# urbste/MultiCol-SLAM

Measured on AMD Instinct MI355X. Metric: Mfeatures/s extract+match, 3-cam 754x480 multi-frame, higher is better.
Workload: dtype u8+i32 (images, Hamming) / f64 (omni model)

## Files before the change

multicol-slam_amd/csrc/mcs_fast.hip:

```cpp
#include "mcs_common.h"

#include <algorithm>
#include <cstdio>
#include <cstdlib>

namespace mcs {

#ifndef MCS_FAST_BS
#define MCS_FAST_BS 128
#endif
template <int CW> struct FastGeom {
	static constexpr int kTileX = 4;
	static constexpr int kTilePitch = (CW + kTileX + 3 + 4 + 3) / 4 * 4, kTileRows = CW + 6;
	static constexpr int kScPitch = (CW + 2 + 3) / 4 * 4, kScRows = CW + 2;
};

template <int P, int kTilePitch> struct Ring;
template <int kTilePitch> struct Ring<12, kTilePitch> {
	static __device__ __forceinline__ void diffs(const uint8_t* c, int (&d)[12]) {
		const int v = c[0];
		d[0] = v - c[2 * kTilePitch]; d[1] = v - c[2 * kTilePitch + 1]; d[2] = v - c[kTilePitch + 2]; d[3] = v - c[2];
		d[4] = v - c[-kTilePitch + 2]; d[5] = v - c[-2 * kTilePitch + 1]; d[6] = v - c[-2 * kTilePitch]; d[7] = v - c[-2 * kTilePitch - 1];
		d[8] = v - c[-kTilePitch - 2]; d[9] = v - c[-2]; d[10] = v - c[kTilePitch - 2]; d[11] = v - c[2 * kTilePitch - 1];
	}
};
template <int kTilePitch> struct Ring<8, kTilePitch> {
	static __device__ __forceinline__ void diffs(const uint8_t* c, int (&d)[8]) {
		const int v = c[0];
		d[0] = v - c[kTilePitch]; d[1] = v - c[kTilePitch + 1]; d[2] = v - c[1]; d[3] = v - c[-kTilePitch + 1];
		d[4] = v - c[-kTilePitch]; d[5] = v - c[-kTilePitch - 1]; d[6] = v - c[-1]; d[7] = v - c[kTilePitch - 1];
	}
};
template <int P>
__device__ __forceinline__ int small_ring_pretest(const int (&d)[P], int t) {
	if (P == 8) {
		bool dk = true, br = true;
#pragma unroll
		for (int k = 0; k < 8; ++k) { dk &= d[k] > t; br &= d[k] < -t; }
		return (dk ? 1 : 0) | (br ? 2 : 0);
	}
	constexpr int pa[8] = {0, 2, 4, 6, 1, 3, 5, 7}, pb[8] = {8, 10, 0, 2, 9, 11, 1, 3};
	bool dk = true, br = true;
#pragma unroll
	for (int i = 0; i < 8; ++i) {
		dk &= (d[pa[i] % P] > t) | (d[pb[i] % P] > t);
		br &= (d[pa[i] % P] < -t) | (d[pb[i] % P] < -t);
	}
	return (dk ? 1 : 0) | (br ? 2 : 0);
}
template <int P, int kTilePitch>
__device__ __forceinline__ bool small_ring_quick(const uint8_t* c, int t) {
	int d[P];
	Ring<P, kTilePitch>::diffs(c, d);
	return small_ring_pretest<P>(d, t) != 0;
}
template <int P, int kTilePitch>
__device__ __forceinline__ int small_ring_score(const uint8_t* c, int t) {
	int d[P];
	Ring<P, kTilePitch>::diffs(c, d);
	const int pre = small_ring_pretest<P>(d, t);
	constexpr int R = P / 2 + 1;
	int A = -256, Bn = 256;
#pragma unroll
	for (int k = 0; k < P; ++k) {
		int lo = d[k], hi = d[k];
#pragma unroll
		for (int j = 1; j < R; ++j) { lo = min(lo, d[(k + j) % P]); hi = max(hi, d[(k + j) % P]); }
		A = max(A, lo);
		Bn = min(Bn, hi);
	}
	const bool corner = ((pre & 1) && A > t) || ((pre & 2) && -Bn > t);
	return corner ? max(A, -Bn) - 1 : 0;
}

template <int AG> struct AgastGeom { static constexpr int P = AG == 0 ? 8 : (AG == 3 ? 16 : 12), N = P / 2 + 1, R = AG == 0 ? 1 : (AG == 2 ? 2 : 3); };
template <int AG, int kTilePitch>
__device__ __forceinline__ int agast_score(const uint8_t* c, int t) {
	constexpr int P = AgastGeom<AG>::P, N = AgastGeom<AG>::N;
	int d[P];
	if constexpr (AG == 1) {
		const int v = c[0];
		d[0] = v - c[-3]; d[1] = v - c[kTilePitch - 2]; d[2] = v - c[2 * kTilePitch - 1]; d[3] = v - c[3 * kTilePitch];
		d[4] = v - c[2 * kTilePitch + 1]; d[5] = v - c[kTilePitch + 2]; d[6] = v - c[3]; d[7] = v - c[-kTilePitch + 2];
		d[8] = v - c[-2 * kTilePitch + 1]; d[9] = v - c[-3 * kTilePitch]; d[10] = v - c[-2 * kTilePitch - 1]; d[11] = v - c[-kTilePitch - 2];
	} else Ring<P, kTilePitch>::diffs(c, d);
	int A = -256, Bn = 256;
#pragma unroll
	for (int k = 0; k < P; ++k) {
		int lo = d[k], hi = d[k];
#pragma unroll
		for (int j = 1; j < N; ++j) { lo = min(lo, d[(k + j) % P]); hi = max(hi, d[(k + j) % P]); }
		A = max(A, lo);
		Bn = min(Bn, hi);
	}
	const int best = max(A, -Bn);
	return best > t ? best - 1 : 0;
}
template <int kTilePitch>
__device__ __forceinline__ bool fast_quick(const uint8_t* c, int t) {
	const int v = c[0];
	const int d0 = v - c[3 * kTilePitch], d8 = v - c[-3 * kTilePitch], d4 = v - c[3], d12 = v - c[-3];
	const bool h0 = d0 > t, h4 = d4 > t, h8 = d8 > t, h12 = d12 > t;
	const bool l0 = d0 < -t, l4 = d4 < -t, l8 = d8 < -t, l12 = d12 < -t;
	return (h0 & h4) | (h4 & h8) | (h8 & h12) | (h12 & h0) | (l0 & l4) | (l4 & l8) | (l8 & l12) | (l12 & l0);
}

typedef short v2s __attribute__((ext_vector_type(2)));
__device__ __forceinline__ v2s as_v2s(uint32_t x) { union { uint32_t u; v2s v; } c; c.u = x; return c.v; }
__device__ __forceinline__ uint32_t as_u32(v2s x) { union { uint32_t u; v2s v; } c; c.v = x; return c.u; }
template <int kTilePitch, int R = 3>
__device__ __forceinline__ uint32_t fast_quick4(const uint8_t* rowc , v2s tt ) {
	const uint32_t A = *reinterpret_cast<const uint32_t*>(rowc - 4), Cc = *reinterpret_cast<const uint32_t*>(rowc), B = *reinterpret_cast<const uint32_t*>(rowc + 4);
	const uint32_t U = *reinterpret_cast<const uint32_t*>(rowc - R * kTilePitch), D = *reinterpret_cast<const uint32_t*>(rowc + R * kTilePitch);
	constexpr uint32_t selR0 = 0x0c000c00u | (uint32_t)(R + 2) << 16 | (uint32_t)R, selR1 = 0x0c000c00u | (uint32_t)(R + 3) << 16 | (uint32_t)(R + 1);
	constexpr uint32_t selL0 = 0x0c000c00u | (uint32_t)(6 - R) << 16 | (uint32_t)(4 - R), selL1 = 0x0c000c00u | (uint32_t)(7 - R) << 16 | (uint32_t)(5 - R);
	static_assert(R != 3 || (selR0 == 0x0c050c03u && selR1 == 0x0c060c04u && selL0 == 0x0c030c01u && selL1 == 0x0c040c02u), "selectors of the 16-pixel ring");
	uint32_t sign[2];
#pragma unroll
	for (int h = 0; h < 2; ++h) {
		const uint32_t own = h ? 0x0c030c01u : 0x0c020c00u;
		const v2s v = as_v2s(__builtin_amdgcn_perm(0u, Cc, own));
		const v2s r0 = as_v2s(__builtin_amdgcn_perm(0u, D, own)), r8 = as_v2s(__builtin_amdgcn_perm(0u, U, own));
		const v2s r4 = as_v2s(__builtin_amdgcn_perm(B, Cc, h ? selR1 : selR0));
		const v2s r12 = as_v2s(__builtin_amdgcn_perm(Cc, A, h ? selL1 : selL0));
		const v2s m1 = __builtin_elementwise_max(__builtin_elementwise_min(r0, r8), __builtin_elementwise_min(r4, r12));
		const v2s m2 = __builtin_elementwise_min(__builtin_elementwise_max(r0, r8), __builtin_elementwise_max(r4, r12));
		const v2s dark = m1 - (v - tt);
		const v2s bright = (v + tt) - m2;
		sign[h] = as_u32(__builtin_elementwise_min(dark, bright));
	}
	return ((sign[0] >> 15) & 0x00010001u) | ((sign[1] >> 14) & 0x00020002u);
}

template <int kTilePitch>
__device__ __forceinline__ int fast_score(const uint8_t* c , int t) {
	const int v = c[0];
	int d[16];
	d[0] = v - c[3 * kTilePitch];
	d[8] = v - c[-3 * kTilePitch];
	d[4] = v - c[3];
	d[12] = v - c[-3];
	d[1] = v - c[3 * kTilePitch + 1];
	d[2] = v - c[2 * kTilePitch + 2];
	d[3] = v - c[1 * kTilePitch + 3];
	d[5] = v - c[-1 * kTilePitch + 3];
	d[6] = v - c[-2 * kTilePitch + 2];
	d[7] = v - c[-3 * kTilePitch + 1];
	d[9] = v - c[-3 * kTilePitch - 1];
	d[10] = v - c[-2 * kTilePitch - 2];
	d[11] = v - c[-1 * kTilePitch - 3];
	d[13] = v - c[1 * kTilePitch - 3];
	d[14] = v - c[2 * kTilePitch - 2];
	d[15] = v - c[3 * kTilePitch - 1];
	int lo2[16], hi2[16], lo4[16], hi4[16];
#pragma unroll
	for (int k = 0; k < 16; ++k) { lo2[k] = min(d[k], d[(k + 1) & 15]); hi2[k] = max(d[k], d[(k + 1) & 15]); }
#pragma unroll
	for (int k = 0; k < 16; ++k) { lo4[k] = min(lo2[k], lo2[(k + 2) & 15]); hi4[k] = max(hi2[k], hi2[(k + 2) & 15]); }
	int A = -256, Bn = 256;
#pragma unroll
	for (int k = 0; k < 16; ++k) {
		int lo9 = min(min(lo4[k], lo4[(k + 4) & 15]), d[(k + 8) & 15]);
		int hi9 = max(max(hi4[k], hi4[(k + 4) & 15]), d[(k + 8) & 15]);
		A = max(A, lo9);
		Bn = min(Bn, hi9);
	}
	const int best = max(A, -Bn);
	return best > t ? best - 1 : 0;
}

template <int kTilePitch>
__device__ __forceinline__ uint32_t fast_score2(const uint8_t* ca, const uint8_t* cb, int t) {
	auto pk = [&](int off) { v2s r; r.x = (short)ca[off]; r.y = (short)cb[off]; return r; };
	const v2s v = pk(0);
	v2s d[16];
	d[0] = v - pk(3 * kTilePitch);
	d[8] = v - pk(-3 * kTilePitch);
	d[4] = v - pk(3);
	d[12] = v - pk(-3);
	d[1] = v - pk(3 * kTilePitch + 1);
	d[2] = v - pk(2 * kTilePitch + 2);
	d[3] = v - pk(1 * kTilePitch + 3);
	d[5] = v - pk(-1 * kTilePitch + 3);
	d[6] = v - pk(-2 * kTilePitch + 2);
	d[7] = v - pk(-3 * kTilePitch + 1);
	d[9] = v - pk(-3 * kTilePitch - 1);
	d[10] = v - pk(-2 * kTilePitch - 2);
	d[11] = v - pk(-1 * kTilePitch - 3);
	d[13] = v - pk(1 * kTilePitch - 3);
	d[14] = v - pk(2 * kTilePitch - 2);
	d[15] = v - pk(3 * kTilePitch - 1);
	v2s lo2[8], hi2[8], lo4[8], hi4[8];
#pragma unroll
	for (int j = 0; j < 8; ++j) { lo2[j] = __builtin_elementwise_min(d[2 * j + 1], d[(2 * j + 2) & 15]); hi2[j] = __builtin_elementwise_max(d[2 * j + 1], d[(2 * j + 2) & 15]); }
#pragma unroll
	for (int j = 0; j < 8; ++j) { lo4[j] = __builtin_elementwise_min(lo2[j], lo2[(j + 1) & 7]); hi4[j] = __builtin_elementwise_max(hi2[j], hi2[(j + 1) & 7]); }
	v2s A = {-256, -256}, Bn = {256, 256};
#pragma unroll
	for (int j = 0; j < 8; ++j) {
		const v2s a = __builtin_elementwise_min(lo4[j], lo4[(j + 2) & 7]), bb = __builtin_elementwise_max(hi4[j], hi4[(j + 2) & 7]);
		const v2s e0 = d[2 * j], e9 = d[(2 * j + 9) & 15];
		A = __builtin_elementwise_max(A, __builtin_elementwise_min(a, __builtin_elementwise_max(e0, e9)));
		Bn = __builtin_elementwise_min(Bn, __builtin_elementwise_max(bb, __builtin_elementwise_min(e0, e9)));
	}
	const v2s best = __builtin_elementwise_max(A, -Bn);
	const int ba = best.x, bb = best.y;
	return (uint32_t)(ba > t ? ba - 1 : 0) | ((uint32_t)(bb > t ? bb - 1 : 0) << 8);
}

__device__ __forceinline__ int wave_incl_scan(int x) {
	x += __builtin_amdgcn_update_dpp(0, x, 0x111, 0xf, 0xf, false);
	x += __builtin_amdgcn_update_dpp(0, x, 0x112, 0xf, 0xf, false);
	x += __builtin_amdgcn_update_dpp(0, x, 0x114, 0xf, 0xf, false);
	x += __builtin_amdgcn_update_dpp(0, x, 0x118, 0xf, 0xf, false);
	x += __builtin_amdgcn_update_dpp(0, x, 0x142, 0xa, 0xf, false);
	x += __builtin_amdgcn_update_dpp(0, x, 0x143, 0xc, 0xf, false);
	return x;
}

template <int CW, int kFastBS, int P, int AG = -1>
__global__ __launch_bounds__(kFastBS) void k_fast_cells(ExtractBuffers b, int nimg, int nblocks, int perXcd, int cell0, int ncells, unsigned ncellsM) {
	typedef FastGeom<CW> Geo;
	constexpr int kTilePitch = Geo::kTilePitch, kTileRows = Geo::kTileRows, kScPitch = Geo::kScPitch, kScRows = Geo::kScRows;
	constexpr int kTileBytes = (AG >= 0 && 2 * CW * CW > kTileRows * kTilePitch) ? 2 * CW * CW : kTileRows * kTilePitch;
	__shared__ __attribute__((aligned(16))) uint8_t tile[kTileBytes];
	__shared__ __attribute__((aligned(16))) uint8_t sc[(kScRows * kScPitch + 15) / 16 * 16];
	__shared__ uint32_t keepBits[2 * CW];
	__shared__ int rowOff[64];
	__shared__ int runBase;
	__shared__ int nSurv;
	__shared__ unsigned short surv[CW * CW];
	constexpr int QR = AG >= 0 ? AgastGeom<AG < 0 ? 3 : AG>::R : 3;
	constexpr bool kOrdered = P == 16 && AG < 0;
	__shared__ int waveTot[kFastBS / 64];
	int listRun = 0;

	const int logical = (blockIdx.x % kNumXCD) * perXcd + blockIdx.x / kNumXCD;
	if (logical >= nblocks) return;
	const PyrDesc& d = *b.desc;
	const int img = (int)__umulhi((unsigned)logical, ncellsM);
	const int ci = cell0 + (logical - img * ncells);
	const CellInfo cell = b.cells[ci];
	const LevelInfo& L = d.lv[cell.level];
	const int tid = threadIdx.x;
	const int cw = cell.cw, ch = cell.ch;
	int* countOut = b.cellCount + (size_t)img * d.cellsPerImage + ci;
	if (cw <= 0 || ch <= 0) { if (tid == 0) *countOut = 0; return; }

	int stride;
	const uint8_t* src = level_ptr(b, d, img, cell.level, &stride);
	src += (size_t)(cell.y0 - 3) * stride + (cell.x0 - Geo::kTileX);
	const int th = ch + 6;
	const bool stage16 = cell.x0 - Geo::kTileX + kTilePitch <= L.w;
	if (stage16) {
		constexpr int kChunks = (kTilePitch + 15) / 16, kLast = kTilePitch - 16;
		static_assert((kChunks & (kChunks - 1)) == 0 || kChunks == 3 || kChunks == 5 || kChunks == 6, "chunks per row");
		const int nch = kChunks * th;
		for (int c = tid; c < nch; c += kFastBS) {
			const unsigned ty = kChunks == 4 ? (unsigned)c >> 2 : kChunks == 8 ? (unsigned)c >> 3 : (unsigned)c / (unsigned)kChunks;
			const unsigned k = (unsigned)c - ty * (unsigned)kChunks;
			const unsigned xo = min(16u * k, (unsigned)kLast);
			uint4 v;
			__builtin_memcpy(&v, src + (ty * (unsigned)stride + xo), 16);
			uint32_t* dstw = reinterpret_cast<uint32_t*>(&tile[ty * kTilePitch + xo]);
			dstw[0] = v.x; dstw[1] = v.y; dstw[2] = v.z; dstw[3] = v.w;
		}
		for (int i = tid; i < (kScRows * kScPitch + 15) / 16; i += kFastBS) reinterpret_cast<uint4*>(sc)[i] = uint4{0u, 0u, 0u, 0u};
		if (!kOrdered) for (int i = tid; i < 2 * ch; i += kFastBS) keepBits[i] = 0;
		if (tid == 0) { runBase = 0; nSurv = 0; }
		__syncthreads();
	} else {
		const int tw = cw + Geo::kTileX + 3;
		const int ndw = (tw + 3) >> 2;
		const unsigned rowM = (unsigned)cell.rowM;
		const int ndwTile = ndw * th;
		for (int i = tid; i < ndwTile; i += 2 * kFastBS) {
			const int i2 = i + kFastBS;
			const bool has2 = i2 < ndwTile;
			const unsigned ty = ((unsigned)i * rowM) >> 16, kx = (unsigned)i - ty * (unsigned)ndw;
			const unsigned ty2 = ((unsigned)i2 * rowM) >> 16, kx2 = (unsigned)i2 - ty2 * (unsigned)ndw;
			uint32_t v, v2 = 0;
			__builtin_memcpy(&v, src + (ty * (unsigned)stride + 4u * kx), 4);
			if (has2) __builtin_memcpy(&v2, src + (ty2 * (unsigned)stride + 4u * kx2), 4);
			*reinterpret_cast<uint32_t*>(&tile[ty * kTilePitch + 4 * kx]) = v;
			if (has2) *reinterpret_cast<uint32_t*>(&tile[ty2 * kTilePitch + 4 * kx2]) = v2;
		}
		const int sh = ch + 2;
		for (int i = tid; i < sh * (kScPitch / 4); i += kFastBS) reinterpret_cast<uint32_t*>(sc)[i] = 0;
		if (!kOrdered) for (int i = tid; i < 2 * ch; i += kFastBS) keepBits[i] = 0;
		if (tid == 0) { runBase = 0; nSurv = 0; }
		__syncthreads();
	}

	const int t = d.fastThreshold;
	const int lane = tid & 63, wave = tid >> 6;
	if constexpr (P == 16 || AG >= 0) {
		const int segs = (cw + 15) >> 4, nseg = segs * ch;
		const unsigned sM = segs == 1 ? 65536u : segs == 2 ? 32768u : segs == 3 ? 21846u : 16384u;
		const v2s tt = {(short)t, (short)t};
		for (int base = 0; base < nseg; base += kFastBS) {
			const int sg = base + tid;
			uint32_t bits = 0;
			int code = 0;
			if (sg < nseg) {
				const int py = (int)(((unsigned)sg * sM) >> 16), sx = sg - py * segs;
				const uint8_t* rowc = &tile[(py + 3) * kTilePitch + 16 * sx + Geo::kTileX];
				const int valid = cw - 16 * sx;
#pragma unroll
				for (int g = 0; g < 4; ++g) {
					if (4 * g < valid) {
						const uint32_t q = fast_quick4<kTilePitch, QR>(rowc + 4 * g, tt);
						bits |= ((q | (q >> 14)) & 0xFu) << (4 * g);
					}
				}
				if (valid < 16) bits &= (1u << valid) - 1u;
				code = (py << 6) | (16 * sx);
			}
			const int cnt = __popc(bits);
			const int incl = wave_incl_scan(cnt);
			const int total = __builtin_amdgcn_readlane(incl, 63);
			int wbase = 0;
			if constexpr (kOrdered) {
				if (lane == 0) waveTot[wave] = total;
				__syncthreads();
				int before = 0, all = 0;
#pragma unroll
				for (int w = 0; w < kFastBS / 64; ++w) { const int tw_ = waveTot[w]; before += w < wave ? tw_ : 0; all += tw_; }
				wbase = listRun + before;
				listRun += all;
				if (base + kFastBS < nseg) __syncthreads();
			} else if (lane == 0 && total) wbase = atomicAdd(&nSurv, total);
			int pos = __builtin_amdgcn_readfirstlane(wbase) + incl - cnt;
			while (bits) {
				const int j = __builtin_ctz(bits);
				surv[pos++] = (unsigned short)(code + j);
				bits &= bits - 1u;
			}
		}
	} else {
		const int npx = cw * ch;
		const unsigned divM = (262144u + (unsigned)cw - 1u) / (unsigned)cw;
		for (int base = 0; base < npx; base += kFastBS) {
			const int p = base + tid;
			bool pass = false;
			int code = 0;
			if (p < npx) {
				const int py = (int)(((unsigned)p * divM) >> 18), px = p - py * cw;
				pass = small_ring_quick<P, kTilePitch>(&tile[(py + 3) * kTilePitch + px + Geo::kTileX], t);
				code = (py << 6) | px;
			}
			const unsigned long long bal = __ballot(pass);
			int wbase = 0;
			if (lane == 0 && bal) wbase = atomicAdd(&nSurv, __popcll(bal));
			wbase = __shfl(wbase, 0);
			if (pass) surv[wbase + __popcll(bal & ((1ull << lane) - 1ull))] = (unsigned short)code;
		}
	}
	__syncthreads();
	const int ns = kOrdered ? listRun : nSurv;
	if constexpr (P == 16) {
		for (int i = 2 * tid; i < ns; i += 2 * kFastBS) {
			const int pa = surv[i], pb = surv[i + 1 < ns ? i + 1 : i];
			const int ya = pa >> 6, xa = pa & 63, yb = pb >> 6, xb = pb & 63;
			const uint32_t s2 = fast_score2<kTilePitch>(&tile[(ya + 3) * kTilePitch + xa + Geo::kTileX], &tile[(yb + 3) * kTilePitch + xb + Geo::kTileX], t);
			sc[(ya + 1) * kScPitch + xa + 1] = (uint8_t)s2;
			if (i + 1 < ns) sc[(yb + 1) * kScPitch + xb + 1] = (uint8_t)(s2 >> 8);
		}
	} else
		for (int i = tid; i < ns; i += kFastBS) {
			const int p = surv[i];
			const int py = p >> 6, px = p & 63;
			const uint8_t* c = &tile[(py + 3) * kTilePitch + px + Geo::kTileX];
			if constexpr (AG >= 0) sc[(py + 1) * kScPitch + px + 1] = (uint8_t)agast_score<(AG < 0 ? 0 : AG), kTilePitch>(c, t);
			else sc[(py + 1) * kScPitch + px + 1] = (uint8_t)small_ring_score<P, kTilePitch>(c, t);
		}
	__syncthreads();

	uint32_t* slots = b.slots + (size_t)img * d.slotsPerImage + cell.slot;
	const short* mapX = b.maskMap + L.mapX;
	const short* mapY = b.maskMap + L.mapY;
	const uint8_t* mask = b.mask0 ? b.mask0 + (size_t)img * b.mask0Pitch : nullptr;
	if constexpr (AG >= 0) {
		for (int i = tid; i < ns; i += kFastBS) {
			const int p = surv[i];
			if (sc[((p >> 6) + 1) * kScPitch + (p & 63) + 1]) atomicOr(&keepBits[p >> 5], 1u << (p & 31));
		}
		__syncthreads();
		if (wave == 0) {
			const int v = lane < ch ? __popc(keepBits[2 * lane]) + __popc(keepBits[2 * lane + 1]) : 0;
			const int incl = wave_incl_scan(v);
			rowOff[lane] = incl - v;
			if (lane == 63) runBase = incl;
		}
		__syncthreads();
		auto bit = [&](int code) { return (keepBits[code >> 5] >> (code & 31)) & 1u; };
		auto index = [&](int code) {
			const uint32_t w = keepBits[code >> 5], lowm = (1u << (code & 31)) - 1u;
			return rowOff[code >> 6] + (int)((code & 32) ? __popc(keepBits[(code >> 5) - 1]) + __popc(w & lowm) : __popc(w & lowm));
		};
		unsigned short* codes = reinterpret_cast<unsigned short*>(tile);
		short* flags = reinterpret_cast<short*>(surv);
		for (int i = tid; i < ns; i += kFastBS) {
			const int p = surv[i];
			if (sc[((p >> 6) + 1) * kScPitch + (p & 63) + 1]) codes[index(p)] = (unsigned short)p;
		}
		__syncthreads();
		const int n = runBase;
		for (int i = tid; i < n; i += kFastBS) flags[i] = -1;
		__syncthreads();
		if (wave != 0) return;
		uint32_t* slotsA = b.slots + (size_t)img * d.slotsPerImage + cell.slot;
		const uint8_t* maskA = b.mask0 ? b.mask0 + (size_t)img * b.mask0Pitch : nullptr;
		int run = 0;
		auto emit = [&](bool keep, uint32_t inf) {
			const int px = inf & 63, py = (inf >> 6) & 63;
			if (keep && maskA) keep = maskA[(size_t)(b.maskMap + L.mapY)[cell.y0 + py] * b.mask0Stride + (b.maskMap + L.mapX)[cell.x0 + px]] != 0;
			const unsigned long long bal = __ballot(keep);
			if (keep) slotsA[run + __popcll(bal & ((1ull << lane) - 1ull))] =
				(uint32_t)(cell.x0 + px - kMinBorder) | ((uint32_t)(cell.y0 + py - kMinBorder) << 12) | (((inf >> 12) & 0xffu) << 24);
			run += __popcll(bal);
		};
		auto word = [&](int i) -> uint32_t {
			if (i >= n) return 0u;
			const int p = codes[i], py = p >> 6, px = p & 63;
			const uint32_t s0 = sc[(py + 1) * kScPitch + px + 1];
			return (uint32_t)p | (s0 << 12) | ((px > 0 ? bit(p - 1) : 0u) << 20) | ((py > 0 ? bit(p - 64) : 0u) << 21);
		};
		auto respOf = [&](int q) { return (int)sc[((q >> 6) + 1) * kScPitch + (q & 63) + 1]; };
		auto root = [&](int& w) {
			int f = flags[w], q = codes[w];
			while (f != -1) { w = f; f = flags[w]; q = codes[w]; }
			return respOf(q);
		};
		for (int base = 0; base < n; base += 64) {
			const uint32_t inf = word(base + lane);
			const int ab = (inf >> 21) & 1u ? index((int)(inf & 0xfffu) - 64) : 0;
			unsigned long long act = __ballot(((inf >> 20) & 3u) != 0u);
			while (act) {
				const int l = __builtin_ctzll(act);
				act &= act - 1ull;
				const int cur = base + l;
				const uint32_t ci = __builtin_amdgcn_readlane(inf, l);
				const int cr = (int)((ci >> 12) & 0xffu);
				int maxAbove = -1, respAbove = 0;
				if (ci & (1u << 21)) {
					int w = __builtin_amdgcn_readlane(ab, l);
					const int rw = root(w);
					if (cr < rw) { flags[cur] = (short)w; maxAbove = w; respAbove = rw; }
					else flags[w] = (short)cur;
				}
				if (ci & (1u << 20)) {
					int tl = cur - 1;
					const int rt = root(tl);
					if (maxAbove == -1) {
						if (tl != cur) {
							if (cr < rt) flags[cur] = (short)tl;
							else flags[tl] = (short)cur;
						}
					} else if (tl != maxAbove) {
						if (respAbove < rt) { flags[maxAbove] = (short)tl; flags[cur] = (short)tl; }
						else { flags[tl] = (short)maxAbove; flags[cur] = (short)maxAbove; }
					}
				}
			}
		}
		for (int base = 0; base < n; base += 64) {
			const int i = base + lane;
			emit(i < n && flags[i] == -1, word(i));
		}
		if (lane == 0) *countOut = run;
		return;
	}
	if constexpr (kOrdered) {
		int run = 0;
		for (int base = 0; base < ns; base += kFastBS) {
			const int i = base + tid;
			bool keep = false;
			uint32_t rec = 0;
			if (i < ns) {
				const int p = surv[i];
				const int py = p >> 6, px = p & 63;
				const uint8_t* q = &sc[(py + 1) * kScPitch + px + 1];
				const int s0 = q[0];
				const int nb = max(max(max((int)q[-1], (int)q[1]), max((int)q[-kScPitch - 1], (int)q[-kScPitch])),
				                   max(max((int)q[-kScPitch + 1], (int)q[kScPitch - 1]), max((int)q[kScPitch], (int)q[kScPitch + 1])));
				keep = s0 > nb;
				if (keep && mask) {
					const int mx = mapX[cell.x0 + px], my = mapY[cell.y0 + py];
					keep = mask[(size_t)my * b.mask0Stride + mx] != 0;
				}
				rec = (uint32_t)(cell.x0 + px - kMinBorder) | ((uint32_t)(cell.y0 + py - kMinBorder) << 12) | ((uint32_t)s0 << 24);
			}
			const unsigned long long bal = __ballot(keep);
			if (lane == 0) waveTot[wave] = __popcll(bal);
			__syncthreads();
			int before = 0, all = 0;
#pragma unroll
			for (int w = 0; w < kFastBS / 64; ++w) { const int tw_ = waveTot[w]; before += w < wave ? tw_ : 0; all += tw_; }
			if (keep) slots[run + before + __popcll(bal & ((1ull << lane) - 1ull))] = rec;
			run += all;
			if (base + kFastBS < ns) __syncthreads();
		}
		if (tid == 0) *countOut = run;
		return;
	}
	for (int i = tid; i < ns; i += kFastBS) {
		const int p = surv[i];
		const int py = p >> 6, px = p & 63;
		const uint8_t* q = &sc[(py + 1) * kScPitch + px + 1];
		const int s0 = q[0];
		const int nb = max(max(max((int)q[-1], (int)q[1]), max((int)q[-kScPitch - 1], (int)q[-kScPitch])),
		                   max(max((int)q[-kScPitch + 1], (int)q[kScPitch - 1]), max((int)q[kScPitch], (int)q[kScPitch + 1])));
		bool keep = s0 > nb;
		if (keep && mask) {
			const int mx = mapX[cell.x0 + px], my = mapY[cell.y0 + py];
			keep = mask[(size_t)my * b.mask0Stride + mx] != 0;
		}
		if (keep) atomicOr(&keepBits[p >> 5], 1u << (p & 31));
	}
	__syncthreads();
	if (wave == 0) {
		const int v = lane < ch ? __popc(keepBits[2 * lane]) + __popc(keepBits[2 * lane + 1]) : 0;
		const int incl = wave_incl_scan(v);
		rowOff[lane] = incl - v;
		if (lane == 63) runBase = incl;
	}
	__syncthreads();
	for (int i = tid; i < ns; i += kFastBS) {
		const int p = surv[i];
		const uint32_t w = keepBits[p >> 5];
		if ((w >> (p & 31)) & 1u) {
			const int py = p >> 6, px = p & 63;
			const uint32_t below = (p & 32) ? __popc(keepBits[2 * py]) + __popc(w & ((1u << (p & 31)) - 1u)) : __popc(w & ((1u << (p & 31)) - 1u));
			const int s0 = sc[(py + 1) * kScPitch + px + 1];
			slots[rowOff[py] + (int)below] = (uint32_t)(cell.x0 + px - kMinBorder) | ((uint32_t)(cell.y0 + py - kMinBorder) << 12) | ((uint32_t)s0 << 24);
		}
	}
	if (tid == 0) *countOut = runBase;
}

void launch_fast(const ExtractBuffers& b, const PyrDesc& hd, int nimg, hipStream_t s, int level0, int level1) {
	if (level1 > hd.nlevels) level1 = hd.nlevels;
	if (level0 >= level1) return;
	const int cell0 = hd.lv[level0].cellBase;
	const int cellEnd = level1 < hd.nlevels ? hd.lv[level1].cellBase : hd.cellsPerImage;
	const int ncells = cellEnd - cell0;
	const int nblocks = nimg * ncells;
	if (nblocks <= 0) return;
	const int perXcd = (nblocks + kNumXCD - 1) / kNumXCD;
	int cellMax = 0;
	for (int l = level0; l < level1; ++l) cellMax = std::max(cellMax, std::max(hd.lv[l].wCell, hd.lv[l].hCell));
	const dim3 grid(perXcd * kNumXCD);
	if ((unsigned long long)nblocks * (unsigned long long)ncells >= (1ull << 32)) { fprintf(stderr, "mcs: FAST launch too large (%d blocks)\n", nblocks); abort(); }
	const unsigned ncellsM = (unsigned)(((1ull << 32) + (unsigned long long)ncells - 1ull) / (unsigned long long)ncells);
#define MCS_FAST_LAUNCH(P)                                                                                                                      \
	do {                                                                                                                                        \
		if (cellMax <= 40) hipLaunchKernelGGL((k_fast_cells<40, MCS_FAST_BS, P>), grid, dim3(MCS_FAST_BS), 0, s, b, nimg, nblocks, perXcd, cell0, ncells, ncellsM);     \
		else hipLaunchKernelGGL((k_fast_cells<60, 256, P>), grid, dim3(256), 0, s, b, nimg, nblocks, perXcd, cell0, ncells, ncellsM);                   \
	} while (0)
	if (hd.agast >= 0) {
		const int B = hd.agast == 0 ? 1 : (hd.agast == 2 ? 2 : 3);
		const int cellMaxA = cellMax + 6 - 2 * B;
#define MCS_AGAST_LAUNCH(T)                                                                                                                                              \
		do {                                                                                                                                                                 \
			if (cellMaxA <= 44) hipLaunchKernelGGL((k_fast_cells<44, 128, AgastGeom<T>::P, T>), grid, dim3(128), 0, s, b, nimg, nblocks, perXcd, cell0, ncells, ncellsM);   \
			else hipLaunchKernelGGL((k_fast_cells<64, 256, AgastGeom<T>::P, T>), grid, dim3(256), 0, s, b, nimg, nblocks, perXcd, cell0, ncells, ncellsM);                    \
		} while (0)
		if (hd.agast == 0) MCS_AGAST_LAUNCH(0);
		else if (hd.agast == 1) MCS_AGAST_LAUNCH(1);
		else if (hd.agast == 2) MCS_AGAST_LAUNCH(2);
		else MCS_AGAST_LAUNCH(3);
#undef MCS_AGAST_LAUNCH
		return;
	}
	if (hd.fastRing == 16) MCS_FAST_LAUNCH(16);
	else if (hd.fastRing == 12) MCS_FAST_LAUNCH(12);
	else MCS_FAST_LAUNCH(8);
#undef MCS_FAST_LAUNCH
}

}
```

Before: 141.3.

## Run FAST-16 cells with a single wave and cap the shared survivor list

For the ordered FAST-16 path with cells up to 40 pixels, the kernel now launches 64-thread blocks (one wavefront), so the per-iteration waveTot exchange and block barriers in the candidate-list and NMS compaction loops go away. The survivor list is capped at 1024 entries to cut shared memory and raise occupancy. When the cap would overflow, the kernel scores the leftover candidates in place and later runs NMS over every pixel of the cell. The trade-off is less parallelism per cell and a slower full-cell fallback for very dense cells.

```diff
diff --git a/multicol-slam_amd/csrc/mcs_fast.hip b/multicol-slam_amd/csrc/mcs_fast.hip
--- a/multicol-slam_amd/csrc/mcs_fast.hip
+++ b/multicol-slam_amd/csrc/mcs_fast.hip
@@ -6,9 +6,8 @@
 
 namespace mcs {
 
-#ifndef MCS_FAST_BS
-#define MCS_FAST_BS 128
-#endif
+template <int CW, int P, int AG> struct FastThreads { static constexpr int value = CW > 44 ? 256 : (P == 16 && AG < 0 ? 64 : 128); };
+constexpr int kFastListCap = 1024;
 template <int CW> struct FastGeom {
 	static constexpr int kTileX = 4;
 	static constexpr int kTilePitch = (CW + kTileX + 3 + 4 + 3) / 4 * 4, kTileRows = CW + 6;
@@ -229,11 +228,14 @@
 	__shared__ int rowOff[64];
 	__shared__ int runBase;
 	__shared__ int nSurv;
-	__shared__ unsigned short surv[CW * CW];
 	constexpr int QR = AG >= 0 ? AgastGeom<AG < 0 ? 3 : AG>::R : 3;
 	constexpr bool kOrdered = P == 16 && AG < 0;
+	constexpr bool kOneWave = kOrdered && kFastBS == 64;
+	constexpr int kListCap = kOneWave && kFastListCap < CW * CW ? kFastListCap : CW * CW;
+	__shared__ unsigned short surv[kListCap];
 	__shared__ int waveTot[kFastBS / 64];
 	int listRun = 0;
+	bool incomplete = false;
 
 	const int logical = (blockIdx.x % kNumXCD) * perXcd + blockIdx.x / kNumXCD;
 	if (logical >= nblocks) return;
@@ -267,7 +269,7 @@
 		}
 		for (int i = tid; i < (kScRows * kScPitch + 15) / 16; i += kFastBS) reinterpret_cast<uint4*>(sc)[i] = uint4{0u, 0u, 0u, 0u};
 		if (!kOrdered) for (int i = tid; i < 2 * ch; i += kFastBS) keepBits[i] = 0;
-		if (tid == 0) { runBase = 0; nSurv = 0; }
+		if (!kOrdered && tid == 0) { runBase = 0; nSurv = 0; }
 		__syncthreads();
 	} else {
 		const int tw = cw + Geo::kTileX + 3;
@@ -288,7 +290,7 @@
 		const int sh = ch + 2;
 		for (int i = tid; i < sh * (kScPitch / 4); i += kFastBS) reinterpret_cast<uint32_t*>(sc)[i] = 0;
 		if (!kOrdered) for (int i = tid; i < 2 * ch; i += kFastBS) keepBits[i] = 0;
-		if (tid == 0) { runBase = 0; nSurv = 0; }
+		if (!kOrdered && tid == 0) { runBase = 0; nSurv = 0; }
 		__syncthreads();
 	}
 
@@ -320,7 +322,25 @@
 			const int incl = wave_incl_scan(cnt);
 			const int total = __builtin_amdgcn_readlane(incl, 63);
 			int wbase = 0;
-			if constexpr (kOrdered) {
+			if constexpr (kOneWave) {
+				if (listRun + total > kListCap) {
+					incomplete = true;
+					const uint8_t* crow = &tile[((code >> 6) + 3) * kTilePitch + (code & 63) + Geo::kTileX];
+					uint8_t* srow = &sc[((code >> 6) + 1) * kScPitch + (code & 63) + 1];
+					while (bits) {
+						const int ja = __builtin_ctz(bits);
+						bits &= bits - 1u;
+						const int jb = bits ? __builtin_ctz(bits) : ja;
+						bits &= bits - 1u;
+						const uint32_t s2 = fast_score2<kTilePitch>(crow + ja, crow + jb, t);
+						srow[ja] = (uint8_t)s2;
+						if (jb != ja) srow[jb] = (uint8_t)(s2 >> 8);
+					}
+				} else {
+					wbase = listRun;
+					listRun += total;
+				}
+			} else if constexpr (kOrdered) {
 				if (lane == 0) waveTot[wave] = total;
 				__syncthreads();
 				int before = 0, all = 0;
@@ -473,13 +493,16 @@
 	}
 	if constexpr (kOrdered) {
 		int run = 0;
-		for (int base = 0; base < ns; base += kFastBS) {
+		const int n3 = incomplete ? cw * ch : ns;
+		const unsigned divM = incomplete ? (262144u + (unsigned)cw - 1u) / (unsigned)cw : 0u;
+		for (int base = 0; base < n3; base += kFastBS) {
 			const int i = base + tid;
 			bool keep = false;
 			uint32_t rec = 0;
-			if (i < ns) {
-				const int p = surv[i];
-				const int py = p >> 6, px = p & 63;
+			if (i < n3) {
+				int py, px;
+				if (incomplete) { py = (int)(((unsigned)i * divM) >> 18); px = i - py * cw; }
+				else { const int p = surv[i]; py = p >> 6; px = p & 63; }
 				const uint8_t* q = &sc[(py + 1) * kScPitch + px + 1];
 				const int s0 = q[0];
 				const int nb = max(max(max((int)q[-1], (int)q[1]), max((int)q[-kScPitch - 1], (int)q[-kScPitch])),
@@ -492,14 +515,17 @@
 				rec = (uint32_t)(cell.x0 + px - kMinBorder) | ((uint32_t)(cell.y0 + py - kMinBorder) << 12) | ((uint32_t)s0 << 24);
 			}
 			const unsigned long long bal = __ballot(keep);
-			if (lane == 0) waveTot[wave] = __popcll(bal);
-			__syncthreads();
-			int before = 0, all = 0;
-#pragma unroll
-			for (int w = 0; w < kFastBS / 64; ++w) { const int tw_ = waveTot[w]; before += w < wave ? tw_ : 0; all += tw_; }
+			int before = 0, all = __popcll(bal);
+			if constexpr (!kOneWave) {
+				if (lane == 0) waveTot[wave] = all;
+				__syncthreads();
+				all = 0;
+#pragma unroll
+				for (int w = 0; w < kFastBS / 64; ++w) { const int tw_ = waveTot[w]; before += w < wave ? tw_ : 0; all += tw_; }
+			}
 			if (keep) slots[run + before + __popcll(bal & ((1ull << lane) - 1ull))] = rec;
 			run += all;
-			if (base + kFastBS < ns) __syncthreads();
+			if (!kOneWave && base + kFastBS < n3) __syncthreads();
 		}
 		if (tid == 0) *countOut = run;
 		return;
@@ -555,16 +581,18 @@
 	const unsigned ncellsM = (unsigned)(((1ull << 32) + (unsigned long long)ncells - 1ull) / (unsigned long long)ncells);
 #define MCS_FAST_LAUNCH(P)                                                                                                                      \
 	do {                                                                                                                                        \
-		if (cellMax <= 40) hipLaunchKernelGGL((k_fast_cells<40, MCS_FAST_BS, P>), grid, dim3(MCS_FAST_BS), 0, s, b, nimg, nblocks, perXcd, cell0, ncells, ncellsM);     \
-		else hipLaunchKernelGGL((k_fast_cells<60, 256, P>), grid, dim3(256), 0, s, b, nimg, nblocks, perXcd, cell0, ncells, ncellsM);                   \
+		constexpr int T40 = FastThreads<40, P, -1>::value, T60 = FastThreads<60, P, -1>::value;                                                       \
+		if (cellMax <= 40) hipLaunchKernelGGL((k_fast_cells<40, T40, P>), grid, dim3(T40), 0, s, b, nimg, nblocks, perXcd, cell0, ncells, ncellsM);   \
+		else hipLaunchKernelGGL((k_fast_cells<60, T60, P>), grid, dim3(T60), 0, s, b, nimg, nblocks, perXcd, cell0, ncells, ncellsM);                 \
 	} while (0)
 	if (hd.agast >= 0) {
 		const int B = hd.agast == 0 ? 1 : (hd.agast == 2 ? 2 : 3);
 		const int cellMaxA = cellMax + 6 - 2 * B;
 #define MCS_AGAST_LAUNCH(T)                                                                                                                                              \
 		do {                                                                                                                                                                 \
-			if (cellMaxA <= 44) hipLaunchKernelGGL((k_fast_cells<44, 128, AgastGeom<T>::P, T>), grid, dim3(128), 0, s, b, nimg, nblocks, perXcd, cell0, ncells, ncellsM);   \
-			else hipLaunchKernelGGL((k_fast_cells<64, 256, AgastGeom<T>::P, T>), grid, dim3(256), 0, s, b, nimg, nblocks, perXcd, cell0, ncells, ncellsM);                    \
+			constexpr int T44 = FastThreads<44, AgastGeom<T>::P, T>::value, T64 = FastThreads<64, AgastGeom<T>::P, T>::value;                                                 \
+			if (cellMaxA <= 44) hipLaunchKernelGGL((k_fast_cells<44, T44, AgastGeom<T>::P, T>), grid, dim3(T44), 0, s, b, nimg, nblocks, perXcd, cell0, ncells, ncellsM);   \
+			else hipLaunchKernelGGL((k_fast_cells<64, T64, AgastGeom<T>::P, T>), grid, dim3(T64), 0, s, b, nimg, nblocks, perXcd, cell0, ncells, ncellsM);                    \
 		} while (0)
 		if (hd.agast == 0) MCS_AGAST_LAUNCH(0);
 		else if (hd.agast == 1) MCS_AGAST_LAUNCH(1);
```

Measured after the change: 145.3, median of 6. 1.03x the previous value.
